# Dokumushikun/jittor-clip-fewshot

Measured on AMD Instinct MI355X. Metric: images/sec ViT-B/32 fwd+LoRA-bwd bs=256, higher is better.
Workload: dtype f32; 1 GPU; cfg-2: ViT-B/32 + rank-4 LoRA(q,k,v; 12 text + 12 vision blocks; shipped lora_weights.pkl) + 4 text-prompt tokens; run_lora train step = text tower fwd+bwd on 403 captions + image tower fwd+bwd + 100*cos CE + AdamW; global_batch=256, images_per_rank=256, captions=403, tower_streams=2, text_positions=77, parallelism=dp1

## Files before the change

### include/clipfs.h

```cpp
#ifndef CLIPFS_H
#define CLIPFS_H

#include <stddef.h>
#include <stdint.h>

#ifdef __cplusplus
extern "C" {
#endif

#define CLIPFS_OK 0
#define CLIPFS_EINVAL 1
#define CLIPFS_HIPERR_BASE 1000

#define CLIPFS_ABI_VERSION 2
int clipfs_abi_version(void);
const char* clipfs_source_stamp(void);
const char* clipfs_gemm_source_stamp(void);
const char* clipfs_last_error(void);

typedef struct clipfs_gemm_args {
  size_t struct_size;
  const float* A;
  const float* B;
  float* C;
// ... 111 lines not shown
int clipfs_attention_plan(int direction, int batch, int seq, int heads, int causal, int flags,
                          struct clipfs_attention_plan* plan);
int clipfs_attention_mfma_max_seq(void);
int clipfs_attention_mfma_long_fwd(const float* qkv, float* out, float* lse, int batch, int seq, int heads, int causal,
                                   int chunk_tokens, int run_tiles, void* stream);
int clipfs_attention_mfma_long_bwd(const float* qkv, const float* dout, const float* out, const float* lse, float* dqkv,
                                   float* work, int batch, int seq, int heads, int causal, int chunk_tokens, int run_tiles,
                                   void* stream);
int clipfs_attention_bwd_packed_ok(int seq, int causal);
int clipfs_attention_bwd_packed(const float* qkv, const float* dout, const float* out, const float* lse, float* dqkv,
                                const int32_t* off, int batch, int seq, int heads, void* stream);
int clipfs_attention_fwd_packed(const float* qkv, float* out, float* lse, const int32_t* off, int batch, int seq, int heads,
                                void* stream);
int clipfs_attention_bwd_packed_io(const float* qkv, const float* dout, const float* out, const float* lse, float* dqkv,
                                   const int32_t* off, int batch, int seq, int heads, void* stream);
int clipfs_attention_f16_max_seq(void);
int clipfs_attention_f16_fwd(const void* qkv, int qkv_f16, float* out, void* out16, float* lse, int batch, int seq,
                             int heads, int causal, void* stream);
int clipfs_attention_f16_bwd(const void* qkv, int qkv_f16, const void* dout, int dout_f16, const float* out,
                             const float* lse, float* dqkv, void* dqkv16, float* work, int batch, int seq, int heads,
                             int causal, void* stream);
int clipfs_attention_f16_bwd_packed_ok(int seq, int causal);
int clipfs_attention_f16_bwd_packed(const void* qkv, int qkv_f16, const void* dout, int dout_f16, const float* out,
                                    const float* lse, float* dqkv, void* dqkv16, float* work, const int32_t* off, int batch,
                                    int seq, int heads, void* stream);

int clipfs_lora_down(const float* x, const float* A, float* t, int rows, int width, int r, int nseg,
                     unsigned seg_mask, float p, uint64_t seed, uint32_t stream_base, uint32_t drow0,
                     void* keep_bits, void* stream);
int clipfs_lora_keep_bits_ok(int width, int segw, int r, int nseg);
// ... 198 lines not shown
```

### jittor-clip-fewshot_amd/build.py

```python
from __future__ import annotations

import hashlib
import os
import subprocess
import sys
from concurrent.futures import ThreadPoolExecutor

HERE = os.path.dirname(os.path.abspath(__file__))
CSRC = os.path.join(HERE, "csrc")
INCLUDE = os.path.join(os.path.dirname(HERE), "include")
OUT = os.path.join(HERE, "clipfs", "libclipfs_hip.so")
SOURCES = ["common.hip", "gemm.hip", "gemm_bf16.hip", "gemm_f16.hip", "norm.hip", "attention.hip", "attention_f16.hip", "attention_mfma.hip", "attention_mfma16.hip", "lora.hip", "lora_mfma.hip", "elem.hip", "mta.hip", "views.hip", "crops.hip", "resnet.hip", "bpe.hip", "bias_grad.hip", "prompts.hip", "tower.hip"]
HIPCC = os.environ.get("HIPCC", "/opt/rocm/bin/hipcc")
FLAGS = ["--offload-arch=gfx950", "-O3", "-std=c++17", "-fPIC", "-I", INCLUDE, "-I", CSRC, "-Wall",
         "-Wno-unused-function", "-ffp-contract=off"] + os.environ.get("HIPCC_EXTRA", "").split()


def _newer(target: str, deps) -> bool:
    if not os.path.exists(target):
        return True
    t = os.path.getmtime(target)
    return any(os.path.getmtime(d) > t for d in deps)


def _stamp(paths) -> str:
    h = hashlib.sha256()
    for p in paths:
# ... 55 lines not shown
```

### jittor-clip-fewshot_amd/clipfs/_lib.py

```python
from __future__ import annotations

import ctypes as C
import os

ABI_VERSION = 2

_HERE = os.path.dirname(os.path.abspath(__file__))
_TAG = os.environ.get("CLIPFS_LIB_TAG", "")
LIB_PATH = os.path.join(_HERE, f"libclipfs_hip_{_TAG}.so" if _TAG else "libclipfs_hip.so")

c_f32p = C.c_void_p
c_stream = C.c_void_p


class ClipfsError(RuntimeError):
    pass


class GemmArgs(C.Structure):
    _fields_ = [
        ("struct_size", C.c_size_t),
        ("A", C.c_void_p), ("B", C.c_void_p), ("C", C.c_void_p),
        ("M", C.c_int), ("N", C.c_int), ("K", C.c_int),
        ("lda", C.c_int), ("ldb", C.c_int), ("ldc", C.c_int),
# ... 173 lines not shown
    "clipfs_tower_fwd_rows": (_i, [C.POINTER(Tower), _p, _p, _i, _p, _p, _p]),
    "clipfs_tower_rows_mode": (_i, [C.POINTER(Tower)]),
    "clipfs_tower_bwd": (_i, [C.POINTER(Tower), _p, _i, _p, _p, _i, _p]),
    "clipfs_tower_bwd_sparse": (_i, [C.POINTER(Tower), _p, _p, _p, _i, _p, _p, _i, _p]),
    "clipfs_attention_bwd_packed_ok": (_i, [_i, _i]),
    "clipfs_attention_bwd_packed": (_i, [_p, _p, _p, _p, _p, _p, _i, _i, _i, _p]),
    "clipfs_gather_rows_map": (_i, [_p, _sz, _p, _p, _i, _i, _p]),
    "clipfs_put_rows_map": (_i, [_p, _p, _p, _sz, _i, _i, _p]),
    "clipfs_layernorm_bwd_rows": (_i, [_p, _p, _i, _p, _p, _p, _p, _p, _p, _i, _i, _i, _p]),
    "clipfs_tower_pack_mode": (_i, [C.POINTER(Tower), _i, _i]),
    "clipfs_tower_bwd_packed": (_i, [C.POINTER(Tower), _p, _p, _p, _i, _p, _i, _p, _p, _i, _p]),
    "clipfs_layernorm_fwd_lora_map": (_i, [_p, _i, _p, _p, _p, _p, _p, _p, _i, _i, _f, _p, _p, _i, _i, _u, _f, _u64, _u32, _u32, _p,
                                           _p, _p]),
    "clipfs_attention_fwd_packed": (_i, [_p, _p, _p, _p, _i, _i, _i, _p]),
    "clipfs_attention_bwd_packed_io": (_i, [_p, _p, _p, _p, _p, _p, _i, _i, _i, _p]),
    "clipfs_tower_pack_fwd_mode": (_i, [C.POINTER(Tower), _i, _i]),
    "clipfs_tower_fwd_packed": (_i, [C.POINTER(Tower), _p, _p, _p, _i, _i, _p, _p, _p]),
    "clipfs_tower_bwd_packed_saved": (_i, [C.POINTER(Tower), _p, _p, _p, _i, _p, _i, _p, _p, _i, _p]),
    "clipfs_attention_f16_bwd_packed_ok": (_i, [_i, _i]),
    "clipfs_attention_f16_bwd_packed": (_i, [_p, _i, _p, _i, _p, _p, _p, _p, _p, _p, _i, _i, _i, _p]),
    "clipfs_layernorm_bwd_rows_f16": (_i, [_p, _p, _i, _p, _p, _p, _p, _p, _p, _p, _i, _i, _i, _p]),
}

SCALER_SCALE, SCALER_INV_SCALE, SCALER_FOUND, SCALER_TRACKER, SCALER_STEP, SCALER_SKIPPED = 0, 1, 2, 3, 4, 5
SCALER_INV_SQRT_BC2, SCALER_STEP_SIZE, SCALER_SKIP, SCALER_WORDS = 6, 7, 8, 16


def new_gemm_args() -> GemmArgs:
    g = GemmArgs()
    g.struct_size = C.sizeof(GemmArgs)
# ... 68 lines not shown
```

### jittor-clip-fewshot_amd/csrc/elem.hip

```cpp
#include "common.h"

namespace clipfs {

__global__ __launch_bounds__(256) void vit_fill_special_kernel(float* __restrict__ x, const float* __restrict__ cls,
                                                               const float* __restrict__ pos,
                                                               const float* __restrict__ vpt, int batch, int tokens,
                                                               int n_patch, int n_vpt, int width) {
  const int per_img = (1 + n_vpt) * width;
  const size_t total = (size_t)batch * per_img;
  for (size_t i = (size_t)blockIdx.x * 256 + threadIdx.x; i < total; i += (size_t)gridDim.x * 256) {
    const int b = (int)(i / per_img), rem = (int)(i % per_img);
    const int r = rem / width, c = rem % width;
    if (r == 0)
      x[((size_t)b * tokens) * width + c] = cls[c] + pos[c];
    else
      x[((size_t)b * tokens + n_patch + r) * width + c] = vpt[(size_t)(r - 1) * width + c];
  }
}

__global__ __launch_bounds__(256) void text_embed_kernel(const int64_t* __restrict__ ids, const float* __restrict__ table,
                                                         const float* __restrict__ pos, const float* __restrict__ ctx,
                                                         int n_ctx, float* __restrict__ x, int n, int seq, int width) {
  const int nch = width >> 2;
  const size_t total = (size_t)n * seq * nch;
// ... 546 lines not shown
    si[CLIPFS_SCALER_TRACKER] = 0;
  }
  si[CLIPFS_SCALER_FOUND] = 0;
}

__global__ __launch_bounds__(256) void adamw_scaled_kernel(float* __restrict__ p, const float* __restrict__ g,
                                                           float* __restrict__ m, float* __restrict__ v, size_t n,
                                                           float lr, float b1, float b2, float eps, float wd,
                                                           const float* __restrict__ sf) {
  const size_t i = (size_t)blockIdx.x * 256 + threadIdx.x;
  if (i >= n || reinterpret_cast<const int32_t*>(sf)[CLIPFS_SCALER_SKIP] != 0) return;
  adamw_element(p, g, m, v, i, lr, b1, b2, eps, wd, sf[CLIPFS_SCALER_INV_SQRT_BC2], sf[CLIPFS_SCALER_STEP_SIZE],
                sf[CLIPFS_SCALER_INV_SCALE]);
}

__global__ __launch_bounds__(256) void matmul_small_kernel(const float* __restrict__ A, const float* __restrict__ B,
                                                           float* __restrict__ C, int M, int N, int K, long sam, long sak,
                                                           long sbk, long sbn, float alpha) {
  const size_t i = (size_t)blockIdx.x * 256 + threadIdx.x;
  if (i >= (size_t)M * N) return;
  const int m = (int)(i / N), n = (int)(i % N);
  float acc = 0.f;
  for (int k = 0; k < K; ++k) acc = fmaf(A[m * sam + k * sak], B[k * sbk + n * sbn], acc);
  C[i] = alpha * acc;
}

static inline unsigned grid_for(size_t total) {
  size_t b = (total + 255) / 256;
  return (unsigned)(b < 1 ? 1 : (b > 8192 ? 8192 : b));
}


__global__ __launch_bounds__(1024) void l1_loss_kernel(const float* __restrict__ a, const float* __restrict__ b, size_t n,
                                                       float* __restrict__ loss, float* __restrict__ da, float gscale) {
  __shared__ float red[16];
  const int lane = threadIdx.x & 63, wave = threadIdx.x >> 6;
  const float g = gscale / (float)n;
  float acc = 0.f;
  for (size_t i = threadIdx.x; i < n; i += 1024) {
// ... 241 lines not shown
                     n_ctx, x, n, seq, width);
  return launch_status();
}

extern "C" int clipfs_token_rows_grad(const float* dx, float* dctx, int n, int seq, int width, int n_ctx, int first,
                                      void* stream) {
  CLIPFS_REQUIRE(dx && dctx && n > 0 && n_ctx > 0 && first >= 0 && first + n_ctx <= seq && width > 0, "token_rows_grad: bad args");
  hipLaunchKernelGGL(text_ctx_grad_kernel, dim3((n_ctx * width + 255) / 256), dim3(256), 0, (hipStream_t)stream, dx, dctx,
                     n, seq, width, n_ctx, first);
  return launch_status();
}

extern "C" int clipfs_matmul_small(const float* A, const float* B, float* C, int M, int N, int K, long sam, long sak,
                                   long sbk, long sbn, float alpha, void* stream) {
  CLIPFS_REQUIRE(A && B && C && M > 0 && N > 0 && K > 0, "matmul_small: bad args");
  const size_t total = (size_t)M * N;
  hipLaunchKernelGGL(matmul_small_kernel, dim3((unsigned)((total + 255) / 256)), dim3(256), 0, (hipStream_t)stream, A, B, C,
                     M, N, K, sam, sak, sbk, sbn, alpha);
  return launch_status();
}

extern "C" int clipfs_gather_eot(const float* x, const int64_t* ids, float* out, int32_t* idx_out, int n, int seq,
                                 int width, void* stream) {
  CLIPFS_REQUIRE(x && ids && out && n > 0 && seq > 0 && width > 0, "gather_eot: bad args");
  hipLaunchKernelGGL(gather_eot_kernel, dim3(n), dim3(64), 0, (hipStream_t)stream, x, ids, out, idx_out, seq, width);
  return launch_status();
}

extern "C" int clipfs_scatter_rows(const float* dy, const int32_t* idx, float* dx, int n, int seq, int width,
                                   void* stream) {
  CLIPFS_REQUIRE(dy && idx && dx && n > 0 && seq > 0 && width > 0, "scatter_rows: bad args");
  const size_t total = (size_t)n * seq * width;
  hipLaunchKernelGGL(scatter_rows_kernel, dim3(grid_for(total)), dim3(256), 0, (hipStream_t)stream, dy, idx, dx, n, seq,
// ... 245 lines not shown
```

### jittor-clip-fewshot_amd/csrc/gemm.hip

```cpp
#include "common.h"
#include "gemm_common.h"

#include <stdlib.h>

#include <vector>

#ifdef CLIPFS_ABLATION_BUILD
#define CLIPFS_ABLATE(mask, bit) ((mask) & (bit))
#else
#define CLIPFS_ABLATE(mask, bit) 0
#endif

#ifdef CLIPFS_STAMPS
__device__ unsigned long long clipfs_gemm_stamps[16384 * 6];
#define CLIPFS_STAMP(i)                                                                                     \
  do {                                                                                                      \
    if (threadIdx.x == 0 && blockIdx.x < 16384) {                                                           \
      clipfs_gemm_stamps[blockIdx.x * 6 + (i)] = __builtin_amdgcn_s_memtime();                              \
      if ((i) == 1) clipfs_gemm_stamps[blockIdx.x * 6 + 4] = __builtin_amdgcn_s_memrealtime();              \
      if ((i) == 2) clipfs_gemm_stamps[blockIdx.x * 6 + 5] = __builtin_amdgcn_s_memrealtime();              \
      if (0) {                                                                                       \
        unsigned hw, xcc;                                                                                   \
        asm volatile("s_getreg_b32 %0, hwreg(HW_REG_HW_ID)" : "=s"(hw));                                  \
        asm volatile("s_getreg_b32 %0, hwreg(HW_REG_XCC_ID)" : "=s"(xcc));                                \
// ... 123 lines not shown
      for (int i = 0; i < B_CHUNKS; ++i)
        b_reg[i] = k_ok ? *reinterpret_cast<const f32x4*>(b_src[i] + k) : f32x4{0.f, 0.f, 0.f, 0.f};
    }
  };
  auto store_lds = [&](int stage) __attribute__((always_inline)) {
    float* s = smem + stage * STAGE_FLOATS;
#pragma unroll
    for (int i = 0; i < A_CHUNKS; ++i) *reinterpret_cast<f32x4*>(s + a_lds[i]) = a_reg[i];
#pragma unroll
    for (int i = 0; i < B_CHUNKS; ++i) *reinterpret_cast<f32x4*>(s + b_lds[i]) = b_reg[i];
  };

  const float* ga_src[A_CHUNKS];
  const float* gb_src[B_CHUNKS];
  int ga_lds[A_CHUNKS], gb_lds[B_CHUNKS];
  if (AMODE == 3) {
    const int uw = __builtin_amdgcn_readfirstlane(wave);
#pragma unroll
    for (int i = 0; i < A_CHUNKS; ++i) {
      const int r0 = 8 * (uw + 4 * i), r = r0 + (lane >> 3);
      const int c = (lane & 7) ^ ((r >> 1) & 7);
      ga_src[i] = g.A + (size_t)min(m0 + r, M - 1) * g.lda + 4 * c;
      ga_lds[i] = r0 * BK;
    }
#pragma unroll
    for (int i = 0; i < B_CHUNKS; ++i) {
      const int r0 = 8 * (uw + 4 * i), r = r0 + (lane >> 3);
      const int c = (lane & 7) ^ ((r >> 1) & 7);
      gb_src[i] = g.B + (size_t)min(n0 + r, N - 1) * g.ldb + 4 * c;
      gb_lds[i] = BM * BK + r0 * BK;
    }
  }
  auto glds_stage = [&](int kt, int stage) __attribute__((always_inline)) {
    float* s = smem + stage * STAGE_FLOATS;
    const int k0 = kt * BK;
#pragma unroll
    for (int i = 0; i < A_CHUNKS; ++i) glds16(ga_src[i] + k0, s + ga_lds[i]);
#pragma unroll
    for (int i = 0; i < B_CHUNKS; ++i) glds16(gb_src[i] + k0, s + gb_lds[i]);
  };

  const int fr = lane & 31, fh = lane >> 5;
  const int swz = (fr >> 1) & 7;
  int a_frag[TM], b_frag[TN];
#pragma unroll
  for (int t = 0; t < TM; ++t) a_frag[t] = (wm * (BM / WM) + t * 32 + fr) * BK;
#pragma unroll
  for (int t = 0; t < TN; ++t) b_frag[t] = BM * BK + (wn * (BN / WN) + t * 32 + fr) * BK;

  f32x16 acc[TM][TN];
#pragma unroll
  for (int i = 0; i < TM; ++i)
// ... 16 lines not shown
      for (int t = 0; t < TN; ++t) bv[t] = *reinterpret_cast<const f32x4*>(s + b_frag[t] + ch);
#pragma unroll
      for (int e = 0; e < 4; ++e) {
#pragma unroll
        for (int i = 0; i < TM; ++i) {
          const float ae = av[i][e];
#pragma unroll
          for (int j = 0; j < TN; ++j) {
            const float be = bv[j][e];
            acc[i][j] = __builtin_amdgcn_mfma_f32_32x32x2f32(ae, be, acc[i][j], 0, 0, 0);
          }
        }
      }
    }
  };
  if (AMODE == 3) {
    glds_stage(kt0, 0);
    __syncthreads();
    CLIPFS_STAMP(1);
    for (int kt = 0; kt + 1 < nk; ++kt) {
      glds_stage(kt0 + kt + 1, (kt + 1) & 1);
      compute(smem + (kt & 1) * STAGE_FLOATS);
      __syncthreads();
    }
    compute(smem + ((nk - 1) & 1) * STAGE_FLOATS);
  } else {
  load_global(kt0);
  store_lds(0);
  __syncthreads();
  for (int kt = 0; kt + 1 < nk; ++kt) {
    if (!CLIPFS_ABLATE(p.ablate, 1)) load_global(kt0 + kt + 1);
// ... 48 lines not shown
      for (int i = 0; i < TM; ++i)
#pragma unroll
        for (int j = 0; j < TN; ++j) {
          f32x4 u[4];
#pragma unroll
          for (int v = 0; v < 4; ++v)
            u[v] = __builtin_bit_cast(f32x4, __builtin_amdgcn_raw_buffer_load_b128(
                                                 rs, (((i * TN + j) * 4 + v) * 256 + tid) * 16, 0,  16));
#pragma unroll
          for (int v = 0; v < 4; ++v)
#pragma unroll
            for (int e = 0; e < 4; ++e) acc[i][j][4 * v + e] += u[v][e];
        }
    }
  }
  finish_tiles<TM, TN>(g, p.patches, acc, m0 + wm * (BM / WM), n0 + wn * (BN / WN), m0 + BM <= M && n0 + BN <= N, lane);
  CLIPFS_STAMP(3);
}

struct SkSeg {
  int tile, kb, ke;
};

#ifndef CLIPFS_SK_WAVES
#define CLIPFS_SK_WAVES 2
#endif
template <int BM, int BN, int NSTAGE>
__global__ __launch_bounds__(256, CLIPFS_SK_WAVES) void gemm_sk_kernel(const GemmParams p) {
  extern __shared__ __attribute__((aligned(16))) float smem[];
  constexpr int WM = BM >= 64 ? 2 : 1;
  constexpr int WN = 4 / WM;
// ... 615 lines not shown
    return launch<128, 64, 0>(p, s);
  }
  if (sk_enabled() && tile_cfg == 0 && a.a_mode == 0 && (a.K % BK) == 0 && a.workspace && a.counters &&
      sk_config(a.M, a.N, a.K).use &&
      (long)((a.M + 63) / 64) * ((a.N + 127) / 128) * 2 * (a.K / BK) < (1L << 30) &&
      a.workspace_floats >= clipfs_gemm_workspace_floats(a.M, a.N, a.K) &&
      a.counters_ints >= clipfs_gemm_counter_ints(a.M, a.N, a.K)) {
    CLIPFS_REQUIRE(aligned16(a.workspace), "gemm: workspace must be 16-byte aligned");
    p.splits = 1;
    return launch_sk<64, 128, 2>(p, sk_config(a.M, a.N, a.K).per_cu, s);
  }
  p.n_blocks_n = (a.N + 127) / 128;
  if (gemm_bm(a.M, a.N) == 32 && a.a_mode == 0 && (a.K % BK) == 0) return launch<32, 128, 3>(p, s);
  static const int glds_cfg = getenv("CLIPFS_GEMM_GLDS") ? atoi(getenv("CLIPFS_GEMM_GLDS")) : 1;
  if (a.a_mode == 0 && (a.K % BK) == 0) return glds_cfg ? launch<64, 128, 3>(p, s) : launch<64, 128, 0>(p, s);
  if (a.a_mode == 1 && a.patch == 32 && (a.img_res & 3) == 0) return launch<64, 128, 1>(p, s);
  return launch<64, 128, 2>(p, s);
}
```

### jittor-clip-fewshot_amd/csrc/gemm_common.h

```cpp
#pragma once
#include "common.h"

namespace clipfs {

typedef float f32x16 __attribute__((ext_vector_type(16)));

struct GemmParams {
  clipfs_gemm_args a;
  int n_blocks_n;
  int patches;
  int grid_g;
  int splits;
  float* part;
  int gm;
  int ablate;
  int sk_nk;
  int sk_tile0;
  int sk_dp_rounds;
  int sk_q, sk_r;
  float* sk_part;
  int* sk_cnt;
};

constexpr int BK = 32;
// ... 15 lines not shown
    orow = (size_t)b * g.out_tokens + 1 + pp;
    rrow = (size_t)(1 + pp);
  }
  if (g.act == 1) {
    if (g.aux_out) g.aux_out[orow * g.ldc + n] = v;
    v = quick_gelu(v);
  } else if (g.act == 2) {
    v *= quick_gelu_grad(g.aux_in[orow * g.ldc + n]);
  }
  if (g.residual) v += g.residual[rrow * g.ldres + n];
  if (g.act == 3) v = fmaxf(v, 0.f);
  g.C[orow * g.ldc + n] = v;
}


template <int TM, int TN>
__device__ __forceinline__ void finish_tiles(const clipfs_gemm_args& g, int patches, f32x16 (&acc)[TM][TN], int mw, int nw,
                                             bool full_tile, int lane) {
  const int fr = lane & 31, fh = lane >> 5;
  const int M = g.M, N = g.N;
  const bool lora_mfma = g.lora_t && g.alpha == 1.f;
  if (lora_mfma) {
    const int r = g.lora_r, tw = g.lora_nseg * r;
    const int rsteps = (r + 1) >> 1;
    for (int st = 0; st < rsteps; ++st) {
      const int k = 2 * st + fh;
      const float kmask = k < r ? 1.f : 0.f;
      const int kc2 = min(k, r - 1);
      float bv[TN];
      int segs[TN];
#pragma unroll
// ... 2 lines not shown
        segs[j] = min(nb, N - 1) / g.lora_seg_width;
        bv[j] = g.lora_b[(size_t)min(nb + fr, N - 1) * r + kc2] * kmask;
      }
#pragma unroll
      for (int i = 0; i < TM; ++i) {
        const int m = min(mw + i * 32 + fr, M - 1);
        const float* tp = g.lora_t + (size_t)m * tw + kc2;
#pragma unroll
        for (int j = 0; j < TN; ++j) {
          const float av = g.lora_scale * tp[segs[j] * r];
          acc[i][j] = __builtin_amdgcn_mfma_f32_32x32x2f32(av, bv[j], acc[i][j], 0, 0, 0);
        }
      }
    }
  }
  if (g.a_mode == 0 && full_tile && (lora_mfma || !g.lora_t)) {
    const int ldc = g.ldc;
    const bool pre_res = g.residual != nullptr, pre_aux = !pre_res && g.act == 2;
    float pre[TM][TN][16];
    if (pre_res || pre_aux) {
#pragma unroll
      for (int j = 0; j < TN; ++j)
#pragma unroll
        for (int i = 0; i < TM; ++i) {
          const int mb = mw + i * 32 + 4 * fh, n = nw + j * 32 + fr;
          const float* q = pre_res ? g.residual + (size_t)mb * g.ldres + n : g.aux_in + (size_t)mb * ldc + n;
          const int ldq = pre_res ? g.ldres : ldc;
#pragma unroll
          for (int r = 0; r < 16; ++r) pre[i][j][r] = q[((r & 3) + 8 * (r >> 2)) * ldq];
        }
    }
#pragma unroll
    for (int j = 0; j < TN; ++j) {
      const int n = nw + j * 32 + fr;
      const float bias = g.bias ? g.bias[n] : 0.f;
#pragma unroll
      for (int i = 0; i < TM; ++i) {
        const int mb = mw + i * 32 + 4 * fh;
        const size_t base = (size_t)mb * ldc + n;
        float v[16];
#pragma unroll
        for (int r = 0; r < 16; ++r) v[r] = g.alpha * acc[i][j][r] + bias;
        if (g.act == 1) {
          if (g.aux_out) {
            float* q = g.aux_out + base;
#pragma unroll
            for (int r = 0; r < 16; ++r) q[((r & 3) + 8 * (r >> 2)) * ldc] = v[r];
          }
#pragma unroll
          for (int r = 0; r < 16; ++r) v[r] = quick_gelu(v[r]);
        } else if (g.act == 2) {
          if (pre_aux) {
#pragma unroll
            for (int r = 0; r < 16; ++r) v[r] *= quick_gelu_grad(pre[i][j][r]);
          } else {
            const float* q = g.aux_in + base;
            float u[16];
#pragma unroll
            for (int r = 0; r < 16; ++r) u[r] = q[((r & 3) + 8 * (r >> 2)) * ldc];
#pragma unroll
            for (int r = 0; r < 16; ++r) v[r] *= quick_gelu_grad(u[r]);
          }
        }
        if (pre_res) {
#pragma unroll
          for (int r = 0; r < 16; ++r) v[r] += pre[i][j][r];
        }
        if (g.act == 3) {
#pragma unroll
          for (int r = 0; r < 16; ++r) v[r] = fmaxf(v[r], 0.f);
        }
        float* q = g.C + base;
#pragma unroll
        for (int r = 0; r < 16; ++r) q[((r & 3) + 8 * (r >> 2)) * ldc] = v[r];
      }
    }
    return;
  }
#pragma unroll
  for (int j = 0; j < TN; ++j) {
    const int n = nw + j * 32 + fr;
    if (n >= N) continue;
#pragma unroll
    for (int i = 0; i < TM; ++i) {
#pragma unroll
      for (int r = 0; r < 16; ++r) {
        const int m = mw + i * 32 + (r & 3) + 8 * (r >> 2) + 4 * fh;
        if (m < M) epilogue_store(g, patches, m, n, acc[i][j][r], lora_mfma);
      }
// ... 13 lines not shown
```

### jittor-clip-fewshot_amd/csrc/tower.hip

```cpp
#include "common.h"

#include <stdlib.h>

#pragma clang diagnostic ignored "-Wc++20-designator"

namespace clipfs {

static inline size_t al4(size_t n) { return (n + 3) & ~(size_t)3; }

static inline bool f16_attention(const clipfs_tower* t) {
  return t->weight_format == 2 && t->seq <= clipfs_attention_f16_max_seq();
}
static inline bool qkv_f16(const clipfs_tower* t) {
  return f16_attention(t) && (t->width % 128) == 0 && t->lora_r <= 64;
}

struct Adapters {
  unsigned qkv_mask;
  bool o, fc, pr;
  bool mlp() const { return fc || pr; }
};
static inline Adapters adapters(const clipfs_block& b) {
  return {b.lora_a_qkv ? (b.lora_mask & 7u) : 0u, b.lora_a_o && (b.lora_mask & 8u), b.lora_a_fc && (b.lora_mask & 16u),
          b.lora_a_pr && (b.lora_mask & 32u)};
// ... 390 lines not shown
  if (!t || batch <= 0 || t->struct_size != sizeof(clipfs_tower)) return 0;
  return scratch_layout(t, (size_t)batch * t->seq).total;
}

extern "C" size_t clipfs_tower_counter_ints(const clipfs_tower* t, int batch) {
  if (!t || batch <= 0 || t->struct_size != sizeof(clipfs_tower)) return 0;
  return scratch_layout(t, (size_t)batch * t->seq).counter_ints;
}

static bool last_block_rows_ok(const clipfs_tower* t) {
  static const bool force_dense = getenv("CLIPFS_DENSE_BWD") && atoi(getenv("CLIPFS_DENSE_BWD")) != 0;
  const Adapters ad = adapters(t->blocks[t->layers - 1]);
  return !(force_dense || ad.o || ad.mlp() || t->seq < 8);
}


static int fwd_tail(const Pass& p, const clipfs_block& b, float* sv, const float* att, const float* x_in,
                    const int32_t* rows, float* x) {
  const clipfs_tower* t = p.t;
  const int d = t->width, Ms = p.batch;
  const SavedLayout& SL = p.SL;
  const size_t Md = (size_t)Ms * d;
  float* at = p.scratch + p.SC.big;
  auto take = [&at](size_t floats) { float* q = at; at += floats; return q; };
  float *att_s = take(Md), *xin_s = take(Md), *xmid_s = take(Md), *h2_s = take(Md), *xout_s = take(Md);
  float *g_s = take(4 * Md), *u_s = take(4 * Md), *mean_s = take(al4((size_t)Ms)), *rstd_s = take((size_t)Ms);
  CLIPFS_CHECK(pick_rows(p, rows, att, d, att_s));
  CLIPFS_CHECK(pick_rows(p, rows, x_in, d, xin_s));
  const bool f16m = t->weight_format == 2;
  CLIPFS_CHECK(gemm(p.cx, {.M = Ms, .N = d, .K = d, .A = att_s, .B = b.w_o, .planes = f16m ? nullptr : b.w_o_p, .C = xmid_s,
// ... 215 lines not shown
  CLIPFS_CHECK(ln_bwd(p, dh, sv + SL.x_mid, b.ln2_g, sv + SL.stat2, dx, dx, h16));
  CLIPFS_CHECK(bias_sum(p, dx, n, d, d, b.g_b_o));
  CLIPFS_CHECK(gemm(v.cx, {.M = n, .N = d, .K = d, .A = dx, .B = b.w_o_t, .planes = b.w_o_t_p, .C = datt, .a16_ready = h16,
                           .c16_only = datt_f16(t, b, h16) ? (void*)datt : nullptr}, p.st));
  if (!adapters(b).o) return CLIPFS_OK;
  const GatherSlots gs = gather_slots(p);
  const float *att, *t_o;
  CLIPFS_CHECK(saved_rows(p, sv + SL.att, d, gs.att, &att));
  CLIPFS_CHECK(saved_rows(p, sv + SL.t_o, t->lora_r, gs.t_o, &t_o));
  return lora_bwd_block(p, l, {.dy = dx, .x = att, .tt = t_o, .A = b.lora_a_o, .B = b.lora_b_o, .gA = b.g_lora_a_o,
                               .gB = b.g_lora_b_o, .dx = datt, .nseg = 1, .mask = 1u,
                               .ds = t->dropout_stream0 + 4u * (uint32_t)l + 3});
}

static int bwd_attn_half(const Pass& p, int l, const float* sv, float* dx, void* h16, const float* res_s,
                         const int32_t* rows, int stop_at_input) {
  const clipfs_tower* t = p.t;
  const clipfs_block& b = t->blocks[l];
  const RowView& v = p.v;
  const SavedLayout& SL = p.SL;
  const int n = v.n, d = t->width, r = t->lora_r;
  const unsigned qkv_mask = adapters(b).qkv_mask;
  float* dh = p.scratch + p.SC.h;
  float* datt = p.scratch + p.SC.b1;
  float* dqkv = p.scratch + p.SC.b3;
  const bool f16a = f16_attention(t);
  const bool dy16 = f16a && p.dqkv16 && (!qkv_mask || clipfs_lora_bwd_f16dy_ok(d, d, r, 3));
  if (v.saved_packed())
    CLIPFS_CHECK(clipfs_attention_bwd_packed_io(sv + SL.qkv, datt, sv + SL.att, sv + SL.lse, dqkv, v.off, p.batch, t->seq,
                                                t->heads, p.st));
  else if (v.packed() && f16a)
    CLIPFS_CHECK(clipfs_attention_f16_bwd_packed(sv + SL.qkv, qkv_f16(t), datt, datt_f16(t, b, h16) ? 1 : 0, sv + SL.att,
                                                 sv + SL.lse, dy16 ? nullptr : dqkv, p.dqkv16, dh, v.off, p.batch, t->seq,
                                                 t->heads, p.st));
  else if (v.packed())
    CLIPFS_CHECK(clipfs_attention_bwd_packed(sv + SL.qkv, datt, sv + SL.att, sv + SL.lse, dqkv, v.off, p.batch, t->seq,
                                             t->heads, p.st));
  else if (f16a)
    CLIPFS_CHECK(clipfs_attention_f16_bwd(sv + SL.qkv, qkv_f16(t), datt, datt_f16(t, b, h16) ? 1 : 0, sv + SL.att,
                                          sv + SL.lse, dy16 ? nullptr : dqkv, p.dqkv16, dh, p.batch, t->seq, t->heads,
                                          t->causal, p.st));
  else
    CLIPFS_CHECK(clipfs_attention_bwd(sv + SL.qkv, datt, sv + SL.att, sv + SL.lse, dqkv, dh, p.batch, t->seq, t->heads,
// ... 74 lines not shown

static int tower_bwd(const Pass& p, const float* dxs, const int32_t* rows, float* dx, const float* saved,
                     int stop_at_input) {
  const clipfs_tower* t = p.t;
  CLIPFS_CHECK(check_bwd_weights(t));
  const int seq = t->seq, d = t->width, top = t->layers - 1;
  if (!rows) return bwd_walk(p, dx, saved, stop_at_input, top);
  if (!last_block_rows_ok(t)) {
    CLIPFS_CHECK(clipfs_scatter_rows(dxs, rows, dx, p.batch, seq, d, p.st));
    return bwd_walk(p, dx, saved, stop_at_input, top);
  }
  const float* sv = saved + (size_t)(top - t->grad_lo) * p.SL.total;
  float *dxm_s, *datt_s;
  CLIPFS_CHECK(bwd_head(p, sv, dxs, rows, &dxm_s, &datt_s));
  float* datt = p.scratch + p.SC.b1;
  if (p.v.packed()) {
    float* dxw = packed_x(p);
    hipError_t e = hipMemsetAsync(datt, 0, ((size_t)(dxw - datt) + (size_t)p.v.n * d) * sizeof(float), p.st);
    CLIPFS_REQUIRE(e == hipSuccess, "tower_bwd_packed: memset failed: %s", hipGetErrorString(e));
    CLIPFS_CHECK(clipfs_put_rows_map(datt_s, p.v.eotp, datt, (size_t)d, p.batch, d, p.st));
    CLIPFS_CHECK(clipfs_put_rows_map(dxm_s, p.v.eotp, dxw, (size_t)d, p.batch, d, p.st));
    CLIPFS_CHECK(bwd_attn_half(p, top, sv, dxw, nullptr, nullptr, nullptr, stop_at_input));
  } else {
    CLIPFS_CHECK(clipfs_scatter_rows(datt_s, rows, datt, p.batch, seq, d, p.st));
    CLIPFS_CHECK(bwd_attn_half(p, top, sv, dx, nullptr, dxm_s, rows, stop_at_input));
  }
  if (!needs_dx(t, top, stop_at_input)) return CLIPFS_OK;
  return bwd_walk(p, dx, saved, stop_at_input, top - 1);
}

extern "C" int clipfs_tower_bwd(const clipfs_tower* t, float* dx, int batch, const float* saved, float* scratch,
                                int stop_at_input, void* stream) {
  Pass p;
  CLIPFS_CHECK(begin_pass(&p, "tower_bwd", t, batch, dx && saved && scratch, &stop_at_input, nullptr, 0, scratch, stream));
  return tower_bwd(p, nullptr, nullptr, dx, saved, stop_at_input);
}

extern "C" int clipfs_tower_bwd_sparse(const clipfs_tower* t, const float* dxs, const int32_t* rows, float* dx, int batch,
                                       const float* saved, float* scratch, int stop_at_input, void* stream) {
  Pass p;
// ... 107 lines not shown
```

Before: 4877 images/s.

## Add single-row attention backward, tiled small matmul, and direct-load patch-embed GEMM

Adds a dedicated kernel for the last transformer block's attention backward when only one query row per sequence (EOT/CLS) carries gradient, so the dense datt scatter and full attention backward are skipped. It also rewrites matmul_small as a shared-memory tiled kernel in place of the one-thread-per-output version. A third change gives the patch-embedding GEMM a direct global-to-LDS load mode (AMODE 4) with im2col addressing and a patch-aware epilogue. These are independent ideas that add new code paths, each with its own correctness risk around packed and causal layouts.

```diff
diff --git a/include/clipfs.h b/include/clipfs.h
--- a/include/clipfs.h
+++ b/include/clipfs.h
@@ -149,6 +149,9 @@
                                 void* stream);
 int clipfs_attention_bwd_packed_io(const float* qkv, const float* dout, const float* out, const float* lse, float* dqkv,
                                    const int32_t* off, int batch, int seq, int heads, void* stream);
+int clipfs_attention_row_ok(int seq, int heads, int width);
+int clipfs_attention_row_bwd(const float* qkv, const float* dout, float* dqkv, const int32_t* rows, const int32_t* off,
+                             int qkv_packed, int batch, int seq, int heads, int causal, void* stream);
 int clipfs_attention_f16_max_seq(void);
 int clipfs_attention_f16_fwd(const void* qkv, int qkv_f16, float* out, void* out16, float* lse, int batch, int seq,
                              int heads, int causal, void* stream);
diff --git a/jittor-clip-fewshot_amd/build.py b/jittor-clip-fewshot_amd/build.py
--- a/jittor-clip-fewshot_amd/build.py
+++ b/jittor-clip-fewshot_amd/build.py
@@ -10,7 +10,7 @@
 CSRC = os.path.join(HERE, "csrc")
 INCLUDE = os.path.join(os.path.dirname(HERE), "include")
 OUT = os.path.join(HERE, "clipfs", "libclipfs_hip.so")
-SOURCES = ["common.hip", "gemm.hip", "gemm_bf16.hip", "gemm_f16.hip", "norm.hip", "attention.hip", "attention_f16.hip", "attention_mfma.hip", "attention_mfma16.hip", "lora.hip", "lora_mfma.hip", "elem.hip", "mta.hip", "views.hip", "crops.hip", "resnet.hip", "bpe.hip", "bias_grad.hip", "prompts.hip", "tower.hip"]
+SOURCES = ["common.hip", "gemm.hip", "gemm_bf16.hip", "gemm_f16.hip", "norm.hip", "attention.hip", "attention_f16.hip", "attention_mfma.hip", "attention_mfma16.hip", "attention_row.hip", "lora.hip", "lora_mfma.hip", "elem.hip", "mta.hip", "views.hip", "crops.hip", "resnet.hip", "bpe.hip", "bias_grad.hip", "prompts.hip", "tower.hip"]
 HIPCC = os.environ.get("HIPCC", "/opt/rocm/bin/hipcc")
 FLAGS = ["--offload-arch=gfx950", "-O3", "-std=c++17", "-fPIC", "-I", INCLUDE, "-I", CSRC, "-Wall",
          "-Wno-unused-function", "-ffp-contract=off"] + os.environ.get("HIPCC_EXTRA", "").split()
diff --git a/jittor-clip-fewshot_amd/clipfs/_lib.py b/jittor-clip-fewshot_amd/clipfs/_lib.py
--- a/jittor-clip-fewshot_amd/clipfs/_lib.py
+++ b/jittor-clip-fewshot_amd/clipfs/_lib.py
@@ -211,6 +211,8 @@
                                            _p, _p]),
     "clipfs_attention_fwd_packed": (_i, [_p, _p, _p, _p, _i, _i, _i, _p]),
     "clipfs_attention_bwd_packed_io": (_i, [_p, _p, _p, _p, _p, _p, _i, _i, _i, _p]),
+    "clipfs_attention_row_ok": (_i, [_i, _i, _i]),
+    "clipfs_attention_row_bwd": (_i, [_p, _p, _p, _p, _p, _i, _i, _i, _i, _i, _p]),
     "clipfs_tower_pack_fwd_mode": (_i, [C.POINTER(Tower), _i, _i]),
     "clipfs_tower_fwd_packed": (_i, [C.POINTER(Tower), _p, _p, _p, _i, _i, _p, _p, _p]),
     "clipfs_tower_bwd_packed_saved": (_i, [C.POINTER(Tower), _p, _p, _p, _i, _p, _i, _p, _p, _i, _p]),
diff --git a/jittor-clip-fewshot_amd/csrc/attention_row.hip b/jittor-clip-fewshot_amd/csrc/attention_row.hip
--- /dev/null
+++ b/jittor-clip-fewshot_amd/csrc/attention_row.hip
@@ -0,0 +1,184 @@
+#include "common.h"
+
+namespace clipfs {
+
+typedef float f32x4 __attribute__((ext_vector_type(4)));
+
+constexpr int ROW_THREADS = 256;
+constexpr int ROW_GROUPS = ROW_THREADS / 16;
+
+struct RowSeq {
+  size_t qkv0, out0;
+  int n, nk, qrow;
+};
+__device__ __forceinline__ RowSeq row_seq(const int32_t* __restrict__ rows, const int32_t* __restrict__ off, int qkv_packed,
+                                          int b, int seq, int causal) {
+  RowSeq s;
+  const int o0 = off ? off[b] : b * seq;
+  s.n = off ? min(off[b + 1] - o0, seq) : seq;
+  s.out0 = (size_t)o0;
+  s.qkv0 = (off && !qkv_packed) ? (size_t)b * seq : (size_t)o0;
+  s.qrow = max(0, min(rows[b], s.n - 1));
+  s.nk = causal ? s.qrow + 1 : s.n;
+  return s;
+}
+
+__device__ __forceinline__ float group_sum(float v) {
+  v += __shfl_xor(v, 1, 64);
+  v += __shfl_xor(v, 2, 64);
+  v += __shfl_xor(v, 4, 64);
+  v += __shfl_xor(v, 8, 64);
+  return v;
+}
+__device__ __forceinline__ float dot4(const f32x4 a, const f32x4 b) {
+  float s = (float)a[0] * (float)b[0];
+  s = fma((float)a[1], (float)b[1], s);
+  s = fma((float)a[2], (float)b[2], s);
+  return fma((float)a[3], (float)b[3], s);
+}
+__device__ __forceinline__ float wave_sum64(float v) {
+#pragma unroll
+  for (int m = 1; m < 64; m <<= 1) v += __shfl_xor(v, m, 64);
+  return v;
+}
+__device__ __forceinline__ float wave_max64(float v) {
+#pragma unroll
+  for (int m = 1; m < 64; m <<= 1) v = fmaxf(v, __shfl_xor(v, m, 64));
+  return v;
+}
+
+__device__ __forceinline__ void row_dots(const float* __restrict__ base, size_t ld, int nk, const f32x4 x, int g, int c,
+                                         float scale, float* __restrict__ dst) {
+  for (int j0 = 0; j0 < nk; j0 += 4 * ROW_GROUPS) {
+    f32x4 kv[4];
+#pragma unroll
+    for (int u = 0; u < 4; ++u) {
+      const int j = j0 + u * ROW_GROUPS + g;
+      kv[u] = j < nk ? *reinterpret_cast<const f32x4*>(base + (size_t)j * ld + 4 * c) : f32x4{0.f, 0.f, 0.f, 0.f};
+    }
+#pragma unroll
+    for (int u = 0; u < 4; ++u) {
+      const int j = j0 + u * ROW_GROUPS + g;
+      const float s = group_sum(dot4(x, kv[u])) * scale;
+      if (c == 0 && j < nk) dst[j] = s;
+    }
+  }
+}
+
+__device__ __forceinline__ void weighted_rows(const float* __restrict__ base, size_t ld, int nk, const float* __restrict__ w,
+                                              int g, int c, float* __restrict__ red) {
+  float acc[4] = {0., 0., 0., 0.};
+  for (int j0 = 0; j0 < nk; j0 += 4 * ROW_GROUPS) {
+    f32x4 kv[4];
+#pragma unroll
+    for (int u = 0; u < 4; ++u) {
+      const int j = j0 + u * ROW_GROUPS + g;
+      kv[u] = j < nk ? *reinterpret_cast<const f32x4*>(base + (size_t)j * ld + 4 * c) : f32x4{0.f, 0.f, 0.f, 0.f};
+    }
+#pragma unroll
+    for (int u = 0; u < 4; ++u) {
+      const int j = j0 + u * ROW_GROUPS + g;
+      if (j < nk) {
+        const float wj = w[j];
+#pragma unroll
+        for (int e = 0; e < 4; ++e) acc[e] = fma(wj, (float)kv[u][e], acc[e]);
+      }
+    }
+  }
+#pragma unroll
+  for (int e = 0; e < 4; ++e) red[g * 64 + 4 * c + e] = acc[e];
+}
+__device__ __forceinline__ float reduce_groups(const float* __restrict__ red, int t) {
+  float s = red[t];
+#pragma unroll
+  for (int g = 1; g < ROW_GROUPS; ++g) s += red[g * 64 + t];
+  return (float)s;
+}
+
+__device__ __forceinline__ void softmax_row(float* __restrict__ sc, int nk, int n, int tid) {
+  const int lane = tid & 63;
+  float mf = -INFINITY;
+  for (int j = lane; j < nk; j += 64) mf = fmaxf(mf, (float)sc[j]);
+  const float m = wave_max64(mf);
+  float l = 0.f;
+  for (int j = lane; j < nk; j += 64) l += expf(sc[j] - m);
+  l = wave_sum64(l);
+  __syncthreads();
+  for (int j = tid; j < n; j += ROW_THREADS) {
+    sc[j] = j < nk ? expf(sc[j] - m) / l : 0.f;
+  }
+  __syncthreads();
+}
+
+__global__ __launch_bounds__(ROW_THREADS) void attention_row_bwd_kernel(const float* __restrict__ qkv,
+                                                                        const float* __restrict__ dout, float* __restrict__ dqkv,
+                                                                        const int32_t* __restrict__ rows,
+                                                                        const int32_t* __restrict__ off, int qkv_packed, int seq,
+                                                                        int heads, int causal) {
+  extern __shared__ __attribute__((aligned(16))) float row_smem[];
+  float* red = row_smem;
+  float* pr = row_smem + ROW_GROUPS * 64;
+  float* ds = pr + seq;
+  const int b = blockIdx.x / heads, h = blockIdx.x - b * heads;
+  const int tid = threadIdx.x, g = tid >> 4, c = tid & 15;
+  const size_t d = (size_t)heads * 64, ld = 3 * d;
+  const RowSeq s = row_seq(rows, off, qkv_packed, b, seq, causal);
+  const float* base = qkv + s.qkv0 * ld + (size_t)h * 64;
+  float* obase = dqkv + s.out0 * ld + (size_t)h * 64;
+  const f32x4 q = *reinterpret_cast<const f32x4*>(base + (size_t)s.qrow * ld + 4 * c);
+  const f32x4 dO = *reinterpret_cast<const f32x4*>(dout + (size_t)b * d + (size_t)h * 64 + 4 * c);
+  row_dots(base + d, ld, s.nk, q, g, c, 0.125f, pr);
+  __syncthreads();
+  softmax_row(pr, s.nk, s.n, tid);
+  row_dots(base + 2 * d, ld, s.nk, dO, g, c, 1.f, ds);
+  __syncthreads();
+  const int lane = tid & 63;
+  float D = 0.f;
+  for (int j = lane; j < s.nk; j += 64) D = fma(pr[j], ds[j], D);
+  D = wave_sum64(D);
+  __syncthreads();
+  for (int j = tid; j < s.n; j += ROW_THREADS) ds[j] = j < s.nk ? pr[j] * (ds[j] - D) * 0.125f : 0.f;
+  __syncthreads();
+  weighted_rows(base + d, ld, s.nk, ds, g, c, red);
+  const f32x4 zero = {0.f, 0.f, 0.f, 0.f};
+  for (int j = g; j < s.n; j += ROW_GROUPS) {
+    float* o = obase + (size_t)j * ld + 4 * c;
+    const float dsj = (float)ds[j], pj = (float)pr[j];
+    if (j != s.qrow) *reinterpret_cast<f32x4*>(o) = zero;
+    *reinterpret_cast<f32x4*>(o + d) = f32x4{dsj * q[0], dsj * q[1], dsj * q[2], dsj * q[3]};
+    *reinterpret_cast<f32x4*>(o + 2 * d) = f32x4{pj * dO[0], pj * dO[1], pj * dO[2], pj * dO[3]};
+  }
+  __syncthreads();
+  if (tid < 64) obase[(size_t)s.qrow * ld + tid] = reduce_groups(red, tid);
+}
+
+constexpr int ROW_MAX_SEQ = 4096;
+
+static int row_check(const char* who, bool ptrs, bool aligned, int batch, int seq, int heads) {
+  CLIPFS_REQUIRE(batch > 0 && heads > 0 && seq > 0 && seq <= ROW_MAX_SEQ, "%s: batch %d seq %d heads %d unsupported (seq <= %d)",
+                 who, batch, seq, heads, ROW_MAX_SEQ);
+  CLIPFS_REQUIRE((long)batch * heads < (1L << 31), "%s: batch * heads too large", who);
+  CLIPFS_REQUIRE(ptrs, "%s: null pointer", who);
+  CLIPFS_REQUIRE(aligned, "%s: misaligned pointer", who);
+  return CLIPFS_OK;
+}
+
+}
+
+using namespace clipfs;
+
+extern "C" int clipfs_attention_row_ok(int seq, int heads, int width) {
+  return seq > 0 && seq <= ROW_MAX_SEQ && heads > 0 && width == 64 * heads;
+}
+
+extern "C" int clipfs_attention_row_bwd(const float* qkv, const float* dout, float* dqkv, const int32_t* rows,
+                                        const int32_t* off, int qkv_packed, int batch, int seq, int heads, int causal,
+                                        void* stream) {
+  CLIPFS_CHECK(row_check("attention_row_bwd", qkv && dout && dqkv && rows, aligned16(qkv) && aligned16(dout) && aligned16(dqkv),
+                         batch, seq, heads));
+  CLIPFS_REQUIRE(off || !qkv_packed, "attention_row_bwd: packed q/k/v need the offsets");
+  const size_t lds = (size_t)(ROW_GROUPS * 64 + 2 * seq) * sizeof(float);
+  hipLaunchKernelGGL(attention_row_bwd_kernel, dim3((unsigned)(batch * heads)), dim3(ROW_THREADS), lds, (hipStream_t)stream, qkv,
+                     dout, dqkv, rows, off, qkv_packed, seq, heads, causal);
+  return launch_status();
+}
diff --git a/jittor-clip-fewshot_amd/csrc/elem.hip b/jittor-clip-fewshot_amd/csrc/elem.hip
--- a/jittor-clip-fewshot_amd/csrc/elem.hip
+++ b/jittor-clip-fewshot_amd/csrc/elem.hip
@@ -584,15 +584,58 @@
                 sf[CLIPFS_SCALER_INV_SCALE]);
 }
 
+constexpr int MS_T = 32, MS_KC = 128, MS_LD = MS_T + 2;
 __global__ __launch_bounds__(256) void matmul_small_kernel(const float* __restrict__ A, const float* __restrict__ B,
                                                            float* __restrict__ C, int M, int N, int K, long sam, long sak,
                                                            long sbk, long sbn, float alpha) {
-  const size_t i = (size_t)blockIdx.x * 256 + threadIdx.x;
-  if (i >= (size_t)M * N) return;
-  const int m = (int)(i / N), n = (int)(i % N);
-  float acc = 0.f;
-  for (int k = 0; k < K; ++k) acc = fmaf(A[m * sam + k * sak], B[k * sbk + n * sbn], acc);
-  C[i] = alpha * acc;
+  __shared__ __attribute__((aligned(8))) float as[MS_KC * MS_LD], bs[MS_KC * MS_LD];
+  constexpr int PER = MS_T * MS_KC / 256;
+  const int tid = threadIdx.x, tx = tid & 15, ty = tid >> 4;
+  const int m0 = blockIdx.y * MS_T, n0 = blockIdx.x * MS_T;
+  const bool a_kfast = (sak < 0 ? -sak : sak) <= (sam < 0 ? -sam : sam);
+  const bool b_kfast = (sbk < 0 ? -sbk : sbk) <= (sbn < 0 ? -sbn : sbn);
+  const int a_r0 = a_kfast ? tid / MS_KC : tid % MS_T, a_k0 = a_kfast ? tid % MS_KC : tid / MS_T;
+  const int b_r0 = b_kfast ? tid / MS_KC : tid % MS_T, b_k0 = b_kfast ? tid % MS_KC : tid / MS_T;
+  const int a_dr = a_kfast ? 256 / MS_KC : 0, a_dk = a_kfast ? 0 : 256 / MS_T;
+  const int b_dr = b_kfast ? 256 / MS_KC : 0, b_dk = b_kfast ? 0 : 256 / MS_T;
+  float ar[PER], br[PER];
+  auto fetch = [&](int k0) __attribute__((always_inline)) {
+#pragma unroll
+    for (int i = 0; i < PER; ++i) {
+      const int m = m0 + a_r0 + i * a_dr, n = n0 + b_r0 + i * b_dr, ka = k0 + a_k0 + i * a_dk, kb = k0 + b_k0 + i * b_dk;
+      ar[i] = (m < M && ka < K) ? A[(long)m * sam + (long)ka * sak] : 0.f;
+      br[i] = (n < N && kb < K) ? B[(long)kb * sbk + (long)n * sbn] : 0.f;
+    }
+  };
+  float acc[2][2] = {{0.f, 0.f}, {0.f, 0.f}};
+  fetch(0);
+  for (int k0 = 0; k0 < K; k0 += MS_KC) {
+#pragma unroll
+    for (int i = 0; i < PER; ++i) {
+      as[(a_k0 + i * a_dk) * MS_LD + a_r0 + i * a_dr] = ar[i];
+      bs[(b_k0 + i * b_dk) * MS_LD + b_r0 + i * b_dr] = br[i];
+    }
+    __syncthreads();
+    if (k0 + MS_KC < K) fetch(k0 + MS_KC);
+    const int kn = min(MS_KC, K - k0);
+#pragma unroll 8
+    for (int k = 0; k < kn; ++k) {
+      const float2 a = *reinterpret_cast<const float2*>(as + k * MS_LD + 2 * ty);
+      const float2 b = *reinterpret_cast<const float2*>(bs + k * MS_LD + 2 * tx);
+      acc[0][0] = fmaf(a.x, b.x, acc[0][0]);
+      acc[0][1] = fmaf(a.x, b.y, acc[0][1]);
+      acc[1][0] = fmaf(a.y, b.x, acc[1][0]);
+      acc[1][1] = fmaf(a.y, b.y, acc[1][1]);
+    }
+    __syncthreads();
+  }
+#pragma unroll
+  for (int i = 0; i < 2; ++i)
+#pragma unroll
+    for (int j = 0; j < 2; ++j) {
+      const int m = m0 + 2 * ty + i, n = n0 + 2 * tx + j;
+      if (m < M && n < N) C[(size_t)m * N + n] = alpha * acc[i][j];
+    }
 }
 
 static inline unsigned grid_for(size_t total) {
@@ -864,9 +907,10 @@
 extern "C" int clipfs_matmul_small(const float* A, const float* B, float* C, int M, int N, int K, long sam, long sak,
                                    long sbk, long sbn, float alpha, void* stream) {
   CLIPFS_REQUIRE(A && B && C && M > 0 && N > 0 && K > 0, "matmul_small: bad args");
-  const size_t total = (size_t)M * N;
-  hipLaunchKernelGGL(matmul_small_kernel, dim3((unsigned)((total + 255) / 256)), dim3(256), 0, (hipStream_t)stream, A, B, C,
-                     M, N, K, sam, sak, sbk, sbn, alpha);
+  const unsigned gx = (unsigned)((N + MS_T - 1) / MS_T), gy = (unsigned)((M + MS_T - 1) / MS_T);
+  CLIPFS_REQUIRE(gy <= 65535u, "matmul_small: M %d too large", M);
+  hipLaunchKernelGGL(matmul_small_kernel, dim3(gx, gy), dim3(256), 0, (hipStream_t)stream, A, B, C, M, N, K, sam, sak, sbk,
+                     sbn, alpha);
   return launch_status();
 }
 
diff --git a/jittor-clip-fewshot_amd/csrc/gemm.hip b/jittor-clip-fewshot_amd/csrc/gemm.hip
--- a/jittor-clip-fewshot_amd/csrc/gemm.hip
+++ b/jittor-clip-fewshot_amd/csrc/gemm.hip
@@ -161,13 +161,20 @@
   const float* ga_src[A_CHUNKS];
   const float* gb_src[B_CHUNKS];
   int ga_lds[A_CHUNKS], gb_lds[B_CHUNKS];
-  if (AMODE == 3) {
+  if (AMODE == 3 || AMODE == 4) {
     const int uw = __builtin_amdgcn_readfirstlane(wave);
 #pragma unroll
     for (int i = 0; i < A_CHUNKS; ++i) {
       const int r0 = 8 * (uw + 4 * i), r = r0 + (lane >> 3);
       const int c = (lane & 7) ^ ((r >> 1) & 7);
-      ga_src[i] = g.A + (size_t)min(m0 + r, M - 1) * g.lda + 4 * c;
+      const int m = min(m0 + r, M - 1);
+      if (AMODE == 3) {
+        ga_src[i] = g.A + (size_t)m * g.lda + 4 * c;
+      } else {
+        const int b = m / p.patches, pp = m - b * p.patches;
+        const int py = pp / p.grid_g, px = pp - py * p.grid_g;
+        ga_src[i] = g.A + ((size_t)b * 3 * g.img_res + (size_t)py * g.patch) * g.img_res + (size_t)px * g.patch + 4 * c;
+      }
       ga_lds[i] = r0 * BK;
     }
 #pragma unroll
@@ -181,8 +188,9 @@
   auto glds_stage = [&](int kt, int stage) __attribute__((always_inline)) {
     float* s = smem + stage * STAGE_FLOATS;
     const int k0 = kt * BK;
-#pragma unroll
-    for (int i = 0; i < A_CHUNKS; ++i) glds16(ga_src[i] + k0, s + ga_lds[i]);
+    const size_t ka = AMODE == 4 ? ((size_t)(kt >> 5) * g.img_res + (kt & 31)) * g.img_res : (size_t)k0;
+#pragma unroll
+    for (int i = 0; i < A_CHUNKS; ++i) glds16(ga_src[i] + ka, s + ga_lds[i]);
 #pragma unroll
     for (int i = 0; i < B_CHUNKS; ++i) glds16(gb_src[i] + k0, s + gb_lds[i]);
   };
@@ -229,7 +237,7 @@
       }
     }
   };
-  if (AMODE == 3) {
+  if (AMODE == 3 || AMODE == 4) {
     glds_stage(kt0, 0);
     __syncthreads();
     CLIPFS_STAMP(1);
@@ -308,7 +316,8 @@
         }
     }
   }
-  finish_tiles<TM, TN>(g, p.patches, acc, m0 + wm * (BM / WM), n0 + wn * (BN / WN), m0 + BM <= M && n0 + BN <= N, lane);
+  finish_tiles<TM, TN, AMODE == 4>(g, p.patches, acc, m0 + wm * (BM / WM), n0 + wn * (BN / WN), m0 + BM <= M && n0 + BN <= N,
+                                   lane);
   CLIPFS_STAMP(3);
 }
 
@@ -954,6 +963,7 @@
   if (gemm_bm(a.M, a.N) == 32 && a.a_mode == 0 && (a.K % BK) == 0) return launch<32, 128, 3>(p, s);
   static const int glds_cfg = getenv("CLIPFS_GEMM_GLDS") ? atoi(getenv("CLIPFS_GEMM_GLDS")) : 1;
   if (a.a_mode == 0 && (a.K % BK) == 0) return glds_cfg ? launch<64, 128, 3>(p, s) : launch<64, 128, 0>(p, s);
-  if (a.a_mode == 1 && a.patch == 32 && (a.img_res & 3) == 0) return launch<64, 128, 1>(p, s);
+  if (a.a_mode == 1 && a.patch == 32 && (a.img_res & 3) == 0)
+    return glds_cfg ? launch<64, 128, 4>(p, s) : launch<64, 128, 1>(p, s);
   return launch<64, 128, 2>(p, s);
 }
diff --git a/jittor-clip-fewshot_amd/csrc/gemm_common.h b/jittor-clip-fewshot_amd/csrc/gemm_common.h
--- a/jittor-clip-fewshot_amd/csrc/gemm_common.h
+++ b/jittor-clip-fewshot_amd/csrc/gemm_common.h
@@ -53,7 +53,7 @@
 }
 
 
-template <int TM, int TN>
+template <int TM, int TN, bool PATCH = false>
 __device__ __forceinline__ void finish_tiles(const clipfs_gemm_args& g, int patches, f32x16 (&acc)[TM][TN], int mw, int nw,
                                              bool full_tile, int lane) {
   const int fr = lane & 31, fh = lane >> 5;
@@ -86,8 +86,24 @@
       }
     }
   }
-  if (g.a_mode == 0 && full_tile && (lora_mfma || !g.lora_t)) {
+  if ((PATCH || g.a_mode == 0) && full_tile && (lora_mfma || !g.lora_t)) {
     const int ldc = g.ldc;
+    int crow[PATCH ? TM : 1][16], rrow[PATCH ? TM : 1][16];
+    if (PATCH) {
+#pragma unroll
+      for (int i = 0; i < TM; ++i)
+#pragma unroll
+        for (int r = 0; r < 16; ++r) {
+          const int m = mw + i * 32 + 4 * fh + (r & 3) + 8 * (r >> 2);
+          const int b = m / patches, pp = m - b * patches;
+          crow[i][r] = b * g.out_tokens + 1 + pp;
+          rrow[i][r] = 1 + pp;
+        }
+    }
+    auto at = [&](auto* q, auto* origin, int n, int i, int r, int ld, bool res) __attribute__((always_inline)) -> decltype(q) {
+      if (PATCH) return origin + (size_t)(res ? rrow[i][r] : crow[i][r]) * ld + n;
+      return q + ((r & 3) + 8 * (r >> 2)) * ld;
+    };
     const bool pre_res = g.residual != nullptr, pre_aux = !pre_res && g.act == 2;
     float pre[TM][TN][16];
     if (pre_res || pre_aux) {
@@ -96,10 +112,11 @@
 #pragma unroll
         for (int i = 0; i < TM; ++i) {
           const int mb = mw + i * 32 + 4 * fh, n = nw + j * 32 + fr;
-          const float* q = pre_res ? g.residual + (size_t)mb * g.ldres + n : g.aux_in + (size_t)mb * ldc + n;
+          const float* q0 = pre_res ? g.residual : g.aux_in;
           const int ldq = pre_res ? g.ldres : ldc;
+          const float* q = q0 + (size_t)mb * ldq + n;
 #pragma unroll
-          for (int r = 0; r < 16; ++r) pre[i][j][r] = q[((r & 3) + 8 * (r >> 2)) * ldq];
+          for (int r = 0; r < 16; ++r) pre[i][j][r] = *at(q, q0, n, i, r, ldq, pre_res);
         }
     }
 #pragma unroll
@@ -117,7 +134,7 @@
           if (g.aux_out) {
             float* q = g.aux_out + base;
 #pragma unroll
-            for (int r = 0; r < 16; ++r) q[((r & 3) + 8 * (r >> 2)) * ldc] = v[r];
+            for (int r = 0; r < 16; ++r) *at(q, g.aux_out, n, i, r, ldc, false) = v[r];
           }
 #pragma unroll
           for (int r = 0; r < 16; ++r) v[r] = quick_gelu(v[r]);
@@ -129,7 +146,7 @@
             const float* q = g.aux_in + base;
             float u[16];
 #pragma unroll
-            for (int r = 0; r < 16; ++r) u[r] = q[((r & 3) + 8 * (r >> 2)) * ldc];
+            for (int r = 0; r < 16; ++r) u[r] = *at(q, g.aux_in, n, i, r, ldc, false);
 #pragma unroll
             for (int r = 0; r < 16; ++r) v[r] *= quick_gelu_grad(u[r]);
           }
@@ -144,7 +161,7 @@
         }
         float* q = g.C + base;
 #pragma unroll
-        for (int r = 0; r < 16; ++r) q[((r & 3) + 8 * (r >> 2)) * ldc] = v[r];
+        for (int r = 0; r < 16; ++r) *at(q, g.C, n, i, r, ldc, false) = v[r];
       }
     }
     return;
diff --git a/jittor-clip-fewshot_amd/csrc/tower.hip b/jittor-clip-fewshot_amd/csrc/tower.hip
--- a/jittor-clip-fewshot_amd/csrc/tower.hip
+++ b/jittor-clip-fewshot_amd/csrc/tower.hip
@@ -428,6 +428,10 @@
   return !(force_dense || ad.o || ad.mlp() || t->seq < 8);
 }
 
+static bool last_block_row_attention(const clipfs_tower* t) {
+  return last_block_rows_ok(t) && t->weight_format == 0 && clipfs_attention_row_ok(t->seq, t->heads, t->width);
+}
+
 
 static int fwd_tail(const Pass& p, const clipfs_block& b, float* sv, const float* att, const float* x_in,
                     const int32_t* rows, float* x) {
@@ -673,7 +677,8 @@
 }
 
 static int bwd_attn_half(const Pass& p, int l, const float* sv, float* dx, void* h16, const float* res_s,
-                         const int32_t* rows, int stop_at_input) {
+                         const int32_t* rows, int stop_at_input, const float* datt_row = nullptr,
+                         const int32_t* qrows = nullptr) {
   const clipfs_tower* t = p.t;
   const clipfs_block& b = t->blocks[l];
   const RowView& v = p.v;
@@ -685,7 +690,10 @@
   float* dqkv = p.scratch + p.SC.b3;
   const bool f16a = f16_attention(t);
   const bool dy16 = f16a && p.dqkv16 && (!qkv_mask || clipfs_lora_bwd_f16dy_ok(d, d, r, 3));
-  if (v.saved_packed())
+  if (datt_row)
+    CLIPFS_CHECK(clipfs_attention_row_bwd(sv + SL.qkv, datt_row, dqkv, qrows, v.off, v.saved_packed(), p.batch, t->seq,
+                                          t->heads, t->causal, p.st));
+  else if (v.saved_packed())
     CLIPFS_CHECK(clipfs_attention_bwd_packed_io(sv + SL.qkv, datt, sv + SL.att, sv + SL.lse, dqkv, v.off, p.batch, t->seq,
                                                 t->heads, p.st));
   else if (v.packed() && f16a)
@@ -790,16 +798,18 @@
   float *dxm_s, *datt_s;
   CLIPFS_CHECK(bwd_head(p, sv, dxs, rows, &dxm_s, &datt_s));
   float* datt = p.scratch + p.SC.b1;
+  const float* datt_row = last_block_row_attention(t) ? datt_s : nullptr;
   if (p.v.packed()) {
     float* dxw = packed_x(p);
-    hipError_t e = hipMemsetAsync(datt, 0, ((size_t)(dxw - datt) + (size_t)p.v.n * d) * sizeof(float), p.st);
+    float* zero0 = datt_row ? dxw : datt;
+    hipError_t e = hipMemsetAsync(zero0, 0, ((size_t)(dxw - zero0) + (size_t)p.v.n * d) * sizeof(float), p.st);
     CLIPFS_REQUIRE(e == hipSuccess, "tower_bwd_packed: memset failed: %s", hipGetErrorString(e));
-    CLIPFS_CHECK(clipfs_put_rows_map(datt_s, p.v.eotp, datt, (size_t)d, p.batch, d, p.st));
+    if (!datt_row) CLIPFS_CHECK(clipfs_put_rows_map(datt_s, p.v.eotp, datt, (size_t)d, p.batch, d, p.st));
     CLIPFS_CHECK(clipfs_put_rows_map(dxm_s, p.v.eotp, dxw, (size_t)d, p.batch, d, p.st));
-    CLIPFS_CHECK(bwd_attn_half(p, top, sv, dxw, nullptr, nullptr, nullptr, stop_at_input));
+    CLIPFS_CHECK(bwd_attn_half(p, top, sv, dxw, nullptr, nullptr, nullptr, stop_at_input, datt_row, rows));
   } else {
-    CLIPFS_CHECK(clipfs_scatter_rows(datt_s, rows, datt, p.batch, seq, d, p.st));
-    CLIPFS_CHECK(bwd_attn_half(p, top, sv, dx, nullptr, dxm_s, rows, stop_at_input));
+    if (!datt_row) CLIPFS_CHECK(clipfs_scatter_rows(datt_s, rows, datt, p.batch, seq, d, p.st));
+    CLIPFS_CHECK(bwd_attn_half(p, top, sv, dx, nullptr, dxm_s, rows, stop_at_input, datt_row, rows));
   }
   if (!needs_dx(t, top, stop_at_input)) return CLIPFS_OK;
   return bwd_walk(p, dx, saved, stop_at_input, top - 1);
```

New measurement: 4909 images/s, median of 6. No clear change (+0.7%).
